# RupertLuo/Valley

Hardware: NVIDIA H100
Metric: generated tokens/s (8-frame video requests: ViT-L/14 encode + pool/project + LLaMA prefill + 256 greedy tokens per sequence) (higher is better)
Workload: dtype bf16

## Files before the change

valley_b200/csrc/api.cu:

```cuda
#include <cuda_runtime.h>
#include <cuda.h>

#include <algorithm>
#include <atomic>
#include <cmath>
#include <cstdarg>
#include <cstdio>
#include <cstdlib>
#include <cstring>
#include <map>
#include <memory>
#include <mutex>
#include <string>
#include <type_traits>
#include <utility>
#include <vector>

#include "../../include/valley_b200.h"
#include "attention_tc.cuh"
#include "common.cuh"
#include "gemm_tc.cuh"
#include "simt_kernels.cuh"
#include "decode_kernels.cuh"
#include "decode_mega.cuh"
// ... 166 lines not shown
  Owned<float> part_o;
  Owned<float2> part_ml;
  Owned<unsigned int> counters;
  Owned<float> part_val;
  Owned<int> part_idx;
  Owned<float> logits;
  Owned<long long> cur_tokens;
  Owned<long long> gen_tokens;
  int nsplit = 1;
  Owned<PhaseDesc> d_phases;
  StepParams mega = {};
  size_t mega_smem = 0;
  Owned<long long> dbg;
  Owned<SampleState> d_sample;
  bool sample_dirty = false;
  bool filtered = false;
  bool recording = false;
  Owned<uint32_t> key_bits;
  bool masked = false;
  int mask_words() const { return Smax / 32; }
  Owned<BeamState> d_beam;
  Owned<long long> beam_tok;
  Owned<int> beam_bidx;
  Owned<float> beam_div;
  Owned<int> beam_from;
  Owned<uint8_t> stop_buf, stop_stage;
  cudaEvent_t stop_event = nullptr;
  bool stop_ready = false;
  Owned<int> hist;
  bool procs_ready = false;
  StepGraphs graphs[kStepKinds];
  size_t layer_stride() const { return (size_t)2 * B * ctx->cfg.num_attention_heads * Smax * 128; }
  bf16* k_layer(int l) const { return cache + (size_t)l * layer_stride(); }
  bf16* v_layer(int l) const { return k_layer(l) + layer_stride() / 2; }

  ~vly_kv() {
    if (len_event) cudaEventDestroy(len_event);
    if (stop_event) cudaEventDestroy(stop_event);
  }
};

static int sync_len(vly_kv* kv) {
  if (!kv->len_dirty) return VLY_OK;
  CK(cudaSetDevice(kv->ctx->cfg.device));
  CK(cudaEventSynchronize(kv->len_event));
  kv->host_len = *reinterpret_cast<volatile int*>(kv->h_len.p);
  kv->len_dirty = false;
  return VLY_OK;
}

static inline int cdiv(long long a, long long b) { return int((a + b - 1) / b); }

static std::mutex g_attr_mu;
static std::map<std::pair<int, const void*>, size_t> g_attr_set;
template <typename Kern>
static int ensure_smem_attr(int device, Kern kern, size_t bytes, bool max_carveout) {
  std::lock_guard<std::mutex> lk(g_attr_mu);
  size_t& have = g_attr_set[std::make_pair(device, (const void*)kern)];
  if (bytes > have || (have == 0 && max_carveout)) {
    if (bytes > 0) CK(cudaFuncSetAttribute(kern, cudaFuncAttributeMaxDynamicSharedMemorySize, (int)bytes));
    if (max_carveout) CK(cudaFuncSetAttribute(kern, cudaFuncAttributePreferredSharedMemoryCarveout, 100));
    have = bytes > 0 ? bytes : 1;
  }
  return VLY_OK;
}

static int make_tmap_2d(vly_ctx* c, CUtensorMap* m, const void* ptr, uint64_t inner, uint64_t rows, uint64_t row_stride_bytes,
                        uint32_t box_inner, uint32_t box_rows, bool swizzle128 = true) {
  cuuint64_t dims[2] = {inner, rows};
  cuuint64_t strides[1] = {row_stride_bytes};
  cuuint32_t box[2] = {box_inner, box_rows};
  cuuint32_t es[2] = {1, 1};
  CUresult r = c->encode(m, CU_TENSOR_MAP_DATA_TYPE_BFLOAT16, 2, const_cast<void*>(ptr), dims, strides, box, es,
                         CU_TENSOR_MAP_INTERLEAVE_NONE, swizzle128 ? CU_TENSOR_MAP_SWIZZLE_128B : CU_TENSOR_MAP_SWIZZLE_NONE,
                         CU_TENSOR_MAP_L2_PROMOTION_L2_256B, CU_TENSOR_MAP_FLOAT_OOB_FILL_NONE);
  if (r != CUDA_SUCCESS)
    return fail(VLY_ERR_CUDA, "cuTensorMapEncodeTiled(2d) failed: %d (ptr=%p inner=%llu rows=%llu stride=%llu box=%u,%u)", (int)r, ptr,
                (unsigned long long)inner, (unsigned long long)rows, (unsigned long long)row_stride_bytes, box_inner, box_rows);
  return VLY_OK;
}
static int make_tmap_3d(vly_ctx* c, CUtensorMap* m, const void* ptr, uint64_t d0, uint64_t d1, uint64_t d2, uint64_t s1, uint64_t s2,
                        uint32_t b0, uint32_t b1) {
  cuuint64_t dims[3] = {d0, d1, d2};
  cuuint64_t strides[2] = {s1, s2};
  cuuint32_t box[3] = {b0, b1, 1};
  cuuint32_t es[3] = {1, 1, 1};
  CUresult r = c->encode(m, CU_TENSOR_MAP_DATA_TYPE_BFLOAT16, 3, const_cast<void*>(ptr), dims, strides, box, es,
                         CU_TENSOR_MAP_INTERLEAVE_NONE, CU_TENSOR_MAP_SWIZZLE_128B, CU_TENSOR_MAP_L2_PROMOTION_L2_256B,
                         CU_TENSOR_MAP_FLOAT_OOB_FILL_NONE);
  if (r != CUDA_SUCCESS) return fail(VLY_ERR_CUDA, "cuTensorMapEncodeTiled(3d) failed: %d", (int)r);
  return VLY_OK;
}

static bool pdl_enabled() {
  static const bool on = getenv("VLY_NO_PDL") == nullptr;
  return on;
}
struct LaunchCfg {
  dim3 grid, block;
  size_t smem = 0;
  cudaStream_t st = 0;
  bool pdl = false;
  bool carveout = false;
  bool cooperative = false;
};
template <typename... KArgs, typename... Args>
static int launch(vly_ctx* c, void (*kern)(KArgs...), const LaunchCfg& l, Args&&... args) {
  if (l.smem > 0 || l.carveout) TRY(ensure_smem_attr(c->cfg.device, kern, l.smem, l.carveout));
  cudaLaunchAttribute attr[2];
  unsigned n = 0;
  if (l.pdl && pdl_enabled()) {
    attr[n].id = cudaLaunchAttributeProgrammaticStreamSerialization;
    attr[n++].val.programmaticStreamSerializationAllowed = 1;
  }
  if (l.cooperative) {
    attr[n].id = cudaLaunchAttributeCooperative;
    attr[n++].val.cooperative = 1;
  }
  cudaLaunchConfig_t cfg = {};
  cfg.gridDim = l.grid;
  cfg.blockDim = l.block;
  cfg.dynamicSmemBytes = l.smem;
  cfg.stream = l.st;
  cfg.attrs = attr;
  cfg.numAttrs = n;
  const cudaError_t e = cudaLaunchKernelEx(&cfg, kern, std::forward<Args>(args)...);
  c->launches++;
  if (e != cudaSuccess) {
    cudaGetLastError();
    const char* name = "kernel";
    cudaFuncGetName(&name, (const void*)kern);
    return fail(VLY_ERR_CUDA, "launch of %s failed: %s", name, cudaGetErrorString(e));
  }
  return VLY_OK;
}

static inline int bmax_of(int B) { return B <= 1 ? 1 : (B <= 2 ? 2 : 4); }
template <typename F>
static int with_bmax(int B, F&& f) {
  if (bmax_of(B) == 1) return f(std::integral_constant<int, 1>());
  if (bmax_of(B) == 2) return f(std::integral_constant<int, 2>());
  return f(std::integral_constant<int, 4>());
}
template <typename T>
struct Type { using type = T; };
template <typename F>
static int with_dtype(int dtype, F&& f) {
  if (dtype == VLY_F32) return f(Type<float>());
  if (dtype == VLY_BF16) return f(Type<bf16>());
  if (dtype == VLY_F16) return f(Type<__half>());
  return fail(VLY_ERR_INVALID, "unknown dtype %d", dtype);
}

template <int BN, int EPI>
static int launch_gemm_t(vly_ctx* c, const bf16* A, long long lda, const bf16* W, long long ldw, GemmParams p, cudaStream_t st) {
  using Cfg = GemmCfg<BN>;
  CUtensorMap ta, tb;
  TRY(make_tmap_2d(c, &ta, A, p.K, p.M, lda * 2, 64, 128));
  TRY(make_tmap_2d(c, &tb, W, p.K, p.N, ldw * 2, 64, BN));
  p.num_m_tiles = cdiv(p.M, 128);
  p.num_n_tiles = cdiv(p.N, BN);
  const int tiles = p.num_m_tiles * p.num_n_tiles;
  return launch(c, gemm_tc_kernel<BN, EPI>, {dim3(tiles), dim3(Cfg::THREADS), Cfg::SMEM_BYTES, st, true}, ta, tb, p);
}
template <int EPI>
static int launch_gemm(vly_ctx* c, int bn, const bf16* A, long long lda, const bf16* W, long long ldw, const GemmParams& p,
                       cudaStream_t st) {
  if (bn == 256) return launch_gemm_t<256, EPI>(c, A, lda, W, ldw, p, st);
  return launch_gemm_t<128, EPI>(c, A, lda, W, ldw, p, st);
}
static inline int pick_bn(int N) { return (N % 256 == 0) ? 256 : 128; }
static inline int pick_bn_m(const vly_ctx* c, int N, int M) {
  if (N % 256 != 0) return 128;
  static const int env_bn = getenv("VLY_GEMM_BN") ? atoi(getenv("VLY_GEMM_BN")) : 0;
  if (env_bn == 128 || env_bn == 256) return env_bn;
  const long long t256 = (long long)cdiv(M, 128) * (N / 256), t128 = 2 * t256;
  if (t256 >= 3LL * c->num_sms) return 256;
  const double e256 = (double)t256 / ((double)cdiv(t256, c->num_sms) * c->num_sms);
  const double e128 = (double)t128 / ((double)cdiv(t128, c->num_sms) * c->num_sms);
  return (e128 > e256 * 1.05) ? 128 : 256;
}

__global__ void pack_rows_kernel(const bf16* __restrict__ src, int K, const float* __restrict__ gamma, const float* __restrict__ beta,
                                 const float* __restrict__ bias_in, bf16* __restrict__ dst, int Kdst, int mode, int off,
                                 float* __restrict__ colsum, float* __restrict__ bias_out) {
  __shared__ float r1[8], r2[8];
  const int r = blockIdx.x;
  int dr;
  if (mode == 0) dr = off + r;
  else if (mode == 1) {
    const int h = r >> 7, d = r & 127;
    dr = off + h * 128 + (d < 64 ? 2 * d : 2 * (d - 64) + 1);
  } else dr = 2 * r + off;
  float cs = 0.f, bb = 0.f;
  for (int k = threadIdx.x; k < Kdst; k += blockDim.x) {
    float wf = 0.f;
    if (k < K) {
      const float w = __bfloat162float(src[(size_t)r * K + k]);
      wf = gamma ? bf16_round(w * gamma[k]) : w;
      if (beta) bb += w * beta[k];
    }
    dst[(size_t)dr * Kdst + k] = __float2bfloat16_rn(wf);
    cs += wf;
  }
  cs = warp_sum(cs);
  bb = warp_sum(bb);
  if ((threadIdx.x & 31) == 0) {
    r1[threadIdx.x >> 5] = cs;
    r2[threadIdx.x >> 5] = bb;
  }
  __syncthreads();
  if (threadIdx.x == 0) {
    float a = 0.f, b = 0.f;
    for (int i = 0; i < (int)(blockDim.x >> 5); ++i) {
      a += r1[i];
      b += r2[i];
    }
    if (colsum) colsum[dr] = a;
    if (bias_out) bias_out[dr] = (bias_in ? bias_in[r] : 0.f) + b;
  }
}

__global__ void rope_table_kernel(float2* rope, int max_pos, float theta, int head_dim) {
  const int i = blockIdx.x * blockDim.x + threadIdx.x;
  const int half = head_dim / 2;
  if (i >= max_pos * half) return;
  const int pos = i / half, j = i % half;
  const float inv = 1.0f / powf(theta, float(2 * j) / float(head_dim));
  const float fr = float(pos) * inv;
  rope[i] = make_float2(bf16_round(cosf(fr)), bf16_round(sinf(fr)));
}

__global__ void set_int_kernel(int* p, int v) { *p = v; }

__global__ void __launch_bounds__(128) copy_rows_stats_kernel(const bf16* __restrict__ in, bf16* __restrict__ out,
                                                              float2* __restrict__ stats, int stats_nt, int H) {
  __shared__ float red[4];
  const int row = blockIdx.x;
  float s = 0.f, sq = 0.f;
  for (int c = threadIdx.x * 8; c < H; c += 128 * 8) {
    const uint4 w = *reinterpret_cast<const uint4*>(in + (size_t)row * H + c);
    *reinterpret_cast<uint4*>(out + (size_t)row * H + c) = w;
    const uint32_t ww[4] = {w.x, w.y, w.z, w.w};
#pragma unroll
    for (int i = 0; i < 4; ++i) {
      const float a = bf16_lo(ww[i]), b = bf16_hi(ww[i]);
      s += a + b;
      sq += a * a + b * b;
    }
  }
  s = block_sum_128(s, red);
  sq = block_sum_128(sq, red);
  if (threadIdx.x < stats_nt) stats[(size_t)row * stats_nt + threadIdx.x] = threadIdx.x == 0 ? make_float2(s, sq) : make_float2(0.f, 0.f);
}

__global__ void kv_export_kernel(const bf16* __restrict__ cache, bf16* __restrict__ out, int Smax, int len, int deinterleave) {
  const int bh = blockIdx.y, s = blockIdx.x, c = threadIdx.x;
  const int d = deinterleave ? ((c & 1) ? 64 + (c >> 1) : (c >> 1)) : c;
  out[((size_t)bh * len + s) * 128 + d] = cache[((size_t)bh * Smax + s) * 128 + c];
}

extern "C" int vly_create(const vly_config* cfg, vly_ctx** out) {
  if (!cfg || !out) return fail(VLY_ERR_INVALID, "vly_create: null argument");
  int ndev = 0;
  if (cudaGetDeviceCount(&ndev) != cudaSuccess || ndev == 0)
    return fail(VLY_ERR_CUDA, "vly_create: no CUDA device visible -- this library has no CPU fallback");
  CK(cudaSetDevice(cfg->device));
  cudaDeviceProp prop;
  CK(cudaGetDeviceProperties(&prop, cfg->device));
  if (prop.major != 9) return fail(VLY_ERR_CUDA, "vly_create: device is sm_%d%d; this library is built for sm_90a only", prop.major, prop.minor);
  if (cfg->hidden_size % 128 || cfg->hidden_size / cfg->num_attention_heads != 128)
    return fail(VLY_ERR_INVALID, "vly_create: head_dim must be 128 (hidden %d, heads %d)", cfg->hidden_size, cfg->num_attention_heads);
  if (cfg->intermediate_size % 64) return fail(VLY_ERR_INVALID, "vly_create: intermediate_size must be a multiple of 64");
  if (cfg->vit_hidden != 1024 || cfg->vit_hidden / cfg->vit_heads != 64 || cfg->vit_mlp % 256)
    return fail(VLY_ERR_INVALID, "vly_create: vision tower must be ViT-L width (1024, head_dim 64); the reference hard-codes 1024 (valley_model.py:192)");
  auto c = std::make_unique<vly_ctx>();
  c->cfg = *cfg;
  c->num_sms = prop.multiProcessorCount;
  cudaDriverEntryPointQueryResult qres;
  void* fn = nullptr;
  if (cudaGetDriverEntryPoint("cuTensorMapEncodeTiled", &fn, cudaEnableDefault, &qres) != cudaSuccess || fn == nullptr)
    return fail(VLY_ERR_CUDA, "vly_create: cuTensorMapEncodeTiled entry point not found");
  c->encode = (PFN_encodeTiled)fn;
  if (cudaStreamCreateWithFlags(&c->cap_stream, cudaStreamNonBlocking) != cudaSuccess)
    return fail(VLY_ERR_CUDA, "vly_create: cudaStreamCreate failed");
  *out = c.release();
  return VLY_OK;
}

extern "C" void vly_destroy(vly_ctx* c) {
  if (!c) return;
  cudaSetDevice(c->cfg.device);
  delete c;
}

extern "C" int vly_num_sms(vly_ctx* c, int* out) {
  if (!c || !out) return fail(VLY_ERR_INVALID, "null");
  *out = c->num_sms;
  return VLY_OK;
}
extern "C" int vly_kernel_launch_count(vly_ctx* c, int64_t* out) {
  if (!c || !out) return fail(VLY_ERR_INVALID, "null");
  std::lock_guard<std::mutex> lk(c->mu);
  *out = c->launches;
  return VLY_OK;
}
extern "C" int vly_held_bytes(int64_t* device_bytes, int64_t* pinned_bytes) {
  if (!device_bytes || !pinned_bytes) return fail(VLY_ERR_INVALID, "null");
  *device_bytes = g_held_bytes[0];
  *pinned_bytes = g_held_bytes[1];
  return VLY_OK;
}

static bool ends_with(const std::string& s, const char* suf) {
  const size_t n = strlen(suf);
  return s.size() >= n && s.compare(s.size() - n, n, suf) == 0;
}

extern "C" int vly_load_weight(vly_ctx* c, const char* name, const void* dev_ptr, int dtype, const int64_t* shape, int ndim) {
  if (!c || !name || !dev_ptr || !shape || ndim < 1 || ndim > 4) return fail(VLY_ERR_INVALID, "vly_load_weight: bad argument");
  std::lock_guard<std::mutex> lk(c->mu);
  if (c->finalized) return fail(VLY_ERR_STATE, "vly_load_weight(%s): weights already finalised", name);
  if (dtype != VLY_F32 && dtype != VLY_BF16 && dtype != VLY_F16)
    return fail(VLY_ERR_INVALID, "vly_load_weight(%s): unknown dtype %d", name, dtype);
  CK(cudaSetDevice(c->cfg.device));
  Staged s;
  s.numel = 1;
  for (int i = 0; i < ndim; ++i) {
    s.shape.push_back(shape[i]);
    s.numel *= shape[i];
  }
  const std::string nm(name);
  s.is_f32 = (ndim == 1) || ends_with(nm, "position_embedding.weight");
// ... 1596 lines not shown
```

valley_b200/csrc/gemm_tc.cuh:

```cuda
#pragma once
#include "common.cuh"
#include "wgmma.cuh"

namespace vly {

enum EpiMode : int {
  EPI_BIAS = 0,
  EPI_LN_BIAS = 1,
  EPI_LN_BIAS_GELU = 2,
  EPI_BIAS_RES_STATS = 3,
  EPI_RMS_QKV_ROPE = 4,
  EPI_RMS_SWIGLU = 5,
  EPI_RMS_F32 = 6,
};

struct GemmParams {
  int M, N, K;
  int num_m_tiles, num_n_tiles;
  void* out;
  long long ldo;
  const float* bias;
  const float* colsum;
  const float2* stats_in;
  int stats_in_nt;
  float inv_dim;
  float eps;
  float2* stats_out;
  const __nv_bfloat16* residual;
  long long ldr;
  const float2* rope;
  int S, past, H, nH, Smax;
  __nv_bfloat16* kcache;
  __nv_bfloat16* vcache;
  __nv_bfloat16* peer_out[8];
  int n_peers;
  int peer_tokens, peer_frame_stride;
  long long peer_frame_off;
};

VLY_DEVINL float tanh_approx(float x) {
  float y;
  asm("tanh.approx.f32 %0, %1;" : "=f"(y) : "f"(x));
  return y;
}
VLY_DEVINL float quick_gelu_f(float v) {
  const float h = 0.5f * v;
  return fmaf(h, tanh_approx(0.851f * v), h);
}
VLY_DEVINL float silu_f(float v) {
  const float h = 0.5f * v;
  return fmaf(h, tanh_approx(h), h);
}

template <int BN>
struct GemmCfg {
  static_assert(BN == 128 || BN == 256, "tile width");
  static constexpr int BM = 128, BK = 64;
  static constexpr int STAGES = (BN == 256) ? 4 : 6;
  static constexpr int A_BYTES = BM * BK * 2;
  static constexpr int B_BYTES = BN * BK * 2;
  static constexpr int STAGE_BYTES = A_BYTES + B_BYTES;
  static constexpr int RING_BYTES = STAGES * STAGE_BYTES;
  static constexpr int ACC_LD = BN + 4;
  static_assert(BM * ACC_LD * 4 <= RING_BYTES, "accumulator staging must fit in the drained ring");
  static constexpr int VEC_BYTES = 2  * BN * 4;
  static constexpr int SMEM_BYTES = RING_BYTES + 1024  + 256  + VEC_BYTES;
  static constexpr int THREADS = 384;
};

template <int BN, int EPI>
__global__ void __launch_bounds__(384, 1)
gemm_tc_kernel(const __grid_constant__ CUtensorMap tma_a, const __grid_constant__ CUtensorMap tma_b, const GemmParams p) {
  using Cfg = GemmCfg<BN>;
  constexpr int BM = Cfg::BM, BK = Cfg::BK, STAGES = Cfg::STAGES;
  extern __shared__ uint8_t smem_raw[];
  const uint32_t base_u32 = (smem_u32(smem_raw) + 1023u) & ~1023u;
  uint8_t* smem = smem_raw + (base_u32 - smem_u32(smem_raw));
  uint8_t* sA = smem;
  uint8_t* sB = smem + STAGES * Cfg::A_BYTES;
  uint64_t* bars = reinterpret_cast<uint64_t*>(smem + Cfg::RING_BYTES);
  uint64_t* full_bar = bars;
  uint64_t* empty_bar = bars + STAGES;
  float* sbias = reinterpret_cast<float*>(smem + Cfg::RING_BYTES + 256);
  float* scol = sbias + BN;

  const int wg = threadIdx.x >> 7;
  const int num_kb = (p.K + BK - 1) / BK;
  const int m_blk = (int)blockIdx.x / p.num_n_tiles, n_blk = (int)blockIdx.x % p.num_n_tiles;

  if (threadIdx.x == 0) {
    tma_prefetch_desc(&tma_a);
    tma_prefetch_desc(&tma_b);
    for (int i = 0; i < STAGES; ++i) {
      mbar_init(&full_bar[i], 1);
      mbar_init(&empty_bar[i], 256);
    }
    fence_barrier_init();
  }
  __syncthreads();
  pdl_launch_dependents();

  if (wg == 0) {
    if (threadIdx.x == 0) {
      pdl_wait();
      int stage = 0;
      uint32_t phase = 0;
      for (int kb = 0; kb < num_kb; ++kb) {
        mbar_wait(&empty_bar[stage], phase ^ 1);
        mbar_expect_tx(&full_bar[stage], Cfg::STAGE_BYTES);
        tma_load_2d(sA + stage * Cfg::A_BYTES, &tma_a, &full_bar[stage], kb * BK, m_blk * BM);
        tma_load_2d(sB + stage * Cfg::B_BYTES, &tma_b, &full_bar[stage], kb * BK, n_blk * BN);
        if (++stage == STAGES) { stage = 0; phase ^= 1; }
      }
    }
    return;
  }

  const int ct = threadIdx.x - 128;
  const int t = threadIdx.x & 127;
  const int row0 = (wg - 1) * 64;
  constexpr int NB = BN / 128;
  float acc[NB][64];
#pragma unroll
  for (int nb = 0; nb < NB; ++nb)
#pragma unroll
    for (int i = 0; i < 64; ++i) acc[nb][i] = 0.f;
  {
    int stage = 0, prev = -1;
    uint32_t phase = 0;
    for (int kb = 0; kb < num_kb; ++kb) {
      mbar_wait(&full_bar[stage], phase);
      const uint64_t da = make_smem_desc_sw128(base_u32 + stage * Cfg::A_BYTES + row0 * 128, 16, 1024);
      const uint64_t db = make_smem_desc_sw128(base_u32 + STAGES * Cfg::A_BYTES + stage * Cfg::B_BYTES, 16, 1024);
      wgmma_fence();
#pragma unroll
      for (int k = 0; k < BK / 16; ++k)
#pragma unroll
        for (int nb = 0; nb < NB; ++nb)
          wgmma_ss_n128(acc[nb], da + 2 * k, db + 2 * k + nb * 1024, (kb | k) != 0);
      wgmma_commit();
      wgmma_wait<1>();
      if (prev >= 0) mbar_arrive(&empty_bar[prev]);
      prev = stage;
      if (++stage == STAGES) { stage = 0; phase ^= 1; }
    }
    wgmma_wait<0>();
#pragma unroll
    for (int nb = 0; nb < NB; ++nb) wgmma_fence_regs(acc[nb]);
  }

  pdl_wait();
  constexpr bool kHasVec = (EPI == EPI_BIAS || EPI == EPI_BIAS_RES_STATS || EPI == EPI_LN_BIAS || EPI == EPI_LN_BIAS_GELU);
  if constexpr (kHasVec) {
    for (int i = ct; i < BN; i += 256) {
      const int n = n_blk * BN + i;
      sbias[i] = (p.bias != nullptr && n < p.N) ? __ldg(p.bias + n) : 0.f;
      if constexpr (EPI == EPI_LN_BIAS || EPI == EPI_LN_BIAS_GELU) scol[i] = (n < p.N) ? __ldg(p.colsum + n) : 0.f;
    }
  }
  asm volatile("bar.sync 1, 256;" ::: "memory");
  float* stg = reinterpret_cast<float*>(smem);
  {
    const int w = t >> 5, l = t & 31;
    const int r = row0 + w * 16 + (l >> 2), c0 = (l & 3) * 2;
#pragma unroll
    for (int nb = 0; nb < NB; ++nb)
#pragma unroll
      for (int j = 0; j < 16; ++j) {
        const int col = nb * 128 + j * 8 + c0;
        *reinterpret_cast<float2*>(stg + (size_t)r * Cfg::ACC_LD + col) = make_float2(acc[nb][4 * j], acc[nb][4 * j + 1]);
        *reinterpret_cast<float2*>(stg + (size_t)(r + 8) * Cfg::ACC_LD + col) = make_float2(acc[nb][4 * j + 2], acc[nb][4 * j + 3]);
      }
  }
  asm volatile("bar.sync %0, 128;" ::"r"(1 + wg) : "memory");

  const int r_in_tile = row0 + (t >> 1);
  const int hf = t & 1;
  const int row = m_blk * BM + r_in_tile;
  const bool row_ok = row < p.M;

  float mean = 0.f, rstd = 1.f;
  if constexpr (EPI == EPI_LN_BIAS || EPI == EPI_LN_BIAS_GELU || EPI == EPI_RMS_QKV_ROPE || EPI == EPI_RMS_SWIGLU ||
                EPI == EPI_RMS_F32) {
    if (row_ok) {
      float s = 0.f, ss = 0.f;
      const float2* st = p.stats_in + (size_t)row * p.stats_in_nt;
      for (int i = 0; i < p.stats_in_nt; ++i) {
        const float2 v = st[i];
        s += v.x;
        ss += v.y;
      }
      if constexpr (EPI == EPI_LN_BIAS || EPI == EPI_LN_BIAS_GELU) {
        mean = s * p.inv_dim;
        const float var = fmaxf(ss * p.inv_dim - mean * mean, 0.f);
        rstd = rsqrtf(var + p.eps);
      } else {
        rstd = rsqrtf(ss * p.inv_dim + p.eps);
      }
    }
  }
  int b_idx = 0, pos = 0;
  if constexpr (EPI == EPI_RMS_QKV_ROPE) {
    if (row_ok) {
      b_idx = row / p.S;
      pos = p.past + (row % p.S);
    }
  }
  float st_sum = 0.f, st_sq = 0.f;
  long long peer_row = 0;
  if constexpr (EPI == EPI_BIAS_RES_STATS) {
    if (p.n_peers > 0) {
      const int f = row / p.peer_tokens;
      peer_row = (p.peer_frame_off + (long long)f * p.peer_frame_stride) * p.peer_tokens + (row - f * p.peer_tokens);
    }
  }
  const float* srow = stg + (size_t)r_in_tile * Cfg::ACC_LD;
  auto process_chunk = [&](const int c) {
    const int n0 = n_blk * BN + c * 32;
    if (row_ok && n0 < p.N) {
    float v[32];
#pragma unroll
    for (int i = 0; i < 32; i += 4) {
      const float4 a4 = *reinterpret_cast<const float4*>(srow + c * 32 + i);
      v[i] = a4.x; v[i + 1] = a4.y; v[i + 2] = a4.z; v[i + 3] = a4.w;
    }

    if constexpr (EPI == EPI_BIAS || EPI == EPI_BIAS_RES_STATS) {
      const float4* b4 = reinterpret_cast<const float4*>(sbias + c * 32);
#pragma unroll
      for (int j = 0; j < 8; ++j) {
        const float4 bb = b4[j];
        v[4 * j] += bb.x; v[4 * j + 1] += bb.y; v[4 * j + 2] += bb.z; v[4 * j + 3] += bb.w;
      }
    }
    if constexpr (EPI == EPI_LN_BIAS || EPI == EPI_LN_BIAS_GELU) {
      const float4* b4 = reinterpret_cast<const float4*>(sbias + c * 32);
      const float4* c4 = reinterpret_cast<const float4*>(scol + c * 32);
      const float nm = -mean * rstd;
#pragma unroll
      for (int j = 0; j < 8; ++j) {
        const float4 bb = b4[j], cc = c4[j];
        const float bq[4] = {bb.x, bb.y, bb.z, bb.w}, cq[4] = {cc.x, cc.y, cc.z, cc.w};
#pragma unroll
        for (int t4 = 0; t4 < 4; ++t4) {
          float t = fmaf(rstd, v[4 * j + t4], fmaf(nm, cq[t4], bq[t4]));
          if constexpr (EPI == EPI_LN_BIAS_GELU) t = quick_gelu_f(t);
          v[4 * j + t4] = t;
        }
      }
    }
    if constexpr (EPI == EPI_RMS_QKV_ROPE || EPI == EPI_RMS_SWIGLU || EPI == EPI_RMS_F32) {
#pragma unroll
      for (int i = 0; i < 32; ++i) v[i] *= rstd;
    }

    if constexpr (EPI == EPI_BIAS_RES_STATS) {
      uint4 o[4];
      const uint4* rp = reinterpret_cast<const uint4*>(p.residual + (size_t)row * p.ldr + n0);
#pragma unroll
      for (int j = 0; j < 4; ++j) {
        const uint4 rr = __ldg(rp + j);
        const uint32_t rw[4] = {rr.x, rr.y, rr.z, rr.w};
        uint32_t ow[4];
#pragma unroll
        for (int t = 0; t < 4; ++t) {
          const float a = v[j * 8 + t * 2] + bf16_lo(rw[t]);
          const float b = v[j * 8 + t * 2 + 1] + bf16_hi(rw[t]);
          ow[t] = pack_bf16x2(a, b);
          const float ar = bf16_lo(ow[t]), br = bf16_hi(ow[t]);
          st_sum += ar + br;
          st_sq += ar * ar + br * br;
        }
        o[j] = make_uint4(ow[0], ow[1], ow[2], ow[3]);
      }
      uint4* op = reinterpret_cast<uint4*>(reinterpret_cast<__nv_bfloat16*>(p.out) + (size_t)row * p.ldo + n0);
#pragma unroll
      for (int j = 0; j < 4; ++j) op[j] = o[j];
      if (p.n_peers > 0) {
        for (int q = 0; q < p.n_peers; ++q) {
          uint4* pp = reinterpret_cast<uint4*>(p.peer_out[q] + (size_t)peer_row * p.ldo + n0);
#pragma unroll
          for (int j = 0; j < 4; ++j) pp[j] = o[j];
        }
      }
    } else if constexpr (EPI == EPI_RMS_SWIGLU) {
      uint32_t ow[8];
#pragma unroll
      for (int j = 0; j < 8; ++j) {
        const float a = silu_f(v[4 * j]) * v[4 * j + 1];
        const float b = silu_f(v[4 * j + 2]) * v[4 * j + 3];
        ow[j] = pack_bf16x2(a, b);
      }
      uint4* op = reinterpret_cast<uint4*>(reinterpret_cast<__nv_bfloat16*>(p.out) + (size_t)row * p.ldo + (n0 >> 1));
      op[0] = make_uint4(ow[0], ow[1], ow[2], ow[3]);
      op[1] = make_uint4(ow[4], ow[5], ow[6], ow[7]);
    } else if constexpr (EPI == EPI_RMS_F32) {
      float* op = reinterpret_cast<float*>(p.out) + (size_t)row * p.ldo + n0;
      if (n0 + 32 <= p.N && (p.ldo & 3) == 0) {
#pragma unroll
        for (int j = 0; j < 8; ++j)
          reinterpret_cast<float4*>(op)[j] = make_float4(v[4 * j], v[4 * j + 1], v[4 * j + 2], v[4 * j + 3]);
      } else {
#pragma unroll
        for (int i = 0; i < 32; ++i)
          if (n0 + i < p.N) op[i] = v[i];
      }
    } else if constexpr (EPI == EPI_RMS_QKV_ROPE) {
      const int which = n0 / p.H;
      const int nh = n0 - which * p.H;
      const int head = nh >> 7, cidx = nh & 127;
      if (which < 2) {
        const float2* cs = p.rope + (size_t)pos * 64 + (cidx >> 1);
#pragma unroll
        for (int j = 0; j < 16; ++j) {
          const float2 c_s = __ldg(cs + j);
          const float x0 = v[2 * j], x1 = v[2 * j + 1];
          v[2 * j] = x0 * c_s.x - x1 * c_s.y;
          v[2 * j + 1] = x1 * c_s.x + x0 * c_s.y;
        }
      }
      __nv_bfloat16* dst;
      if (which == 0) {
        dst = reinterpret_cast<__nv_bfloat16*>(p.out) + (size_t)row * p.ldo + nh;
      } else {
        __nv_bfloat16* cache = (which == 1) ? p.kcache : p.vcache;
        dst = cache + (((size_t)b_idx * p.nH + head) * p.Smax + pos) * 128 + cidx;
      }
      uint4* op = reinterpret_cast<uint4*>(dst);
#pragma unroll
      for (int j = 0; j < 4; ++j)
        op[j] = make_uint4(pack_bf16x2(v[8 * j], v[8 * j + 1]), pack_bf16x2(v[8 * j + 2], v[8 * j + 3]),
                           pack_bf16x2(v[8 * j + 4], v[8 * j + 5]), pack_bf16x2(v[8 * j + 6], v[8 * j + 7]));
    } else {
      __nv_bfloat16* dst = reinterpret_cast<__nv_bfloat16*>(p.out) + (size_t)row * p.ldo + n0;
      if (n0 + 32 <= p.N && (p.ldo & 7) == 0) {
        uint4* op = reinterpret_cast<uint4*>(dst);
#pragma unroll
        for (int j = 0; j < 4; ++j)
          op[j] = make_uint4(pack_bf16x2(v[8 * j], v[8 * j + 1]), pack_bf16x2(v[8 * j + 2], v[8 * j + 3]),
                             pack_bf16x2(v[8 * j + 4], v[8 * j + 5]), pack_bf16x2(v[8 * j + 6], v[8 * j + 7]));
      } else {
#pragma unroll
        for (int i = 0; i < 32; ++i)
          if (n0 + i < p.N) dst[i] = __float2bfloat16_rn(v[i]);
      }
    }
    }
  };
  constexpr int CPT = BN / 64;
#pragma unroll
  for (int cc = 0; cc < CPT; ++cc) process_chunk(hf * CPT + cc);
  if constexpr (EPI == EPI_BIAS_RES_STATS) {
    st_sum += __shfl_xor_sync(0xffffffffu, st_sum, 1);
    st_sq += __shfl_xor_sync(0xffffffffu, st_sq, 1);
    if (hf == 0 && row_ok && p.stats_out != nullptr) p.stats_out[(size_t)row * p.num_n_tiles + n_blk] = make_float2(st_sum, st_sq);
  }
}

}
```

Before: 388.2.

## Make tensor-core GEMM persistent with ping-pong consumer warpgroups and banded tile order

```diff
diff --git a/valley_b200/csrc/api.cu b/valley_b200/csrc/api.cu
--- a/valley_b200/csrc/api.cu
+++ b/valley_b200/csrc/api.cu
@@ -342,16 +342,26 @@
   return fail(VLY_ERR_INVALID, "unknown dtype %d", dtype);
 }
 
+static bool gemm_one_tile_per_cta() {
+  const char* e = getenv("VLY_GEMM_ONE_TILE");
+  return e != nullptr && atoi(e) != 0;
+}
+static inline int gemm_tiles(int M, int N, int bn) { return cdiv(M, GemmCfg<128>::BM) * cdiv(N, bn); }
+static inline int gemm_grid(const vly_ctx* c, int tiles) {
+  return gemm_one_tile_per_cta() ? cdiv(tiles, 2) : std::min(tiles, c->num_sms);
+}
 template <int BN, int EPI>
 static int launch_gemm_t(vly_ctx* c, const bf16* A, long long lda, const bf16* W, long long ldw, GemmParams p, cudaStream_t st) {
   using Cfg = GemmCfg<BN>;
   CUtensorMap ta, tb;
-  TRY(make_tmap_2d(c, &ta, A, p.K, p.M, lda * 2, 64, 128));
+  TRY(make_tmap_2d(c, &ta, A, p.K, p.M, lda * 2, 64, Cfg::BM));
   TRY(make_tmap_2d(c, &tb, W, p.K, p.N, ldw * 2, 64, BN));
-  p.num_m_tiles = cdiv(p.M, 128);
+  p.num_m_tiles = cdiv(p.M, Cfg::BM);
   p.num_n_tiles = cdiv(p.N, BN);
-  const int tiles = p.num_m_tiles * p.num_n_tiles;
-  return launch(c, gemm_tc_kernel<BN, EPI>, {dim3(tiles), dim3(Cfg::THREADS), Cfg::SMEM_BYTES, st, true}, ta, tb, p);
+  const long long a_row_block = (long long)Cfg::BM * p.K * 2, a_band = 24LL << 20;
+  p.band_m = (p.M > p.N && p.num_m_tiles * a_row_block > a_band) ? (int)std::max(1LL, a_band / a_row_block) : p.num_m_tiles;
+  const int grid = gemm_grid(c, p.num_m_tiles * p.num_n_tiles);
+  return launch(c, gemm_tc_kernel<BN, EPI>, {dim3(grid), dim3(Cfg::THREADS), Cfg::SMEM_BYTES, st, true}, ta, tb, p);
 }
 template <int EPI>
 static int launch_gemm(vly_ctx* c, int bn, const bf16* A, long long lda, const bf16* W, long long ldw, const GemmParams& p,
@@ -364,11 +374,9 @@
   if (N % 256 != 0) return 128;
   static const int env_bn = getenv("VLY_GEMM_BN") ? atoi(getenv("VLY_GEMM_BN")) : 0;
   if (env_bn == 128 || env_bn == 256) return env_bn;
-  const long long t256 = (long long)cdiv(M, 128) * (N / 256), t128 = 2 * t256;
-  if (t256 >= 3LL * c->num_sms) return 256;
-  const double e256 = (double)t256 / ((double)cdiv(t256, c->num_sms) * c->num_sms);
-  const double e128 = (double)t128 / ((double)cdiv(t128, c->num_sms) * c->num_sms);
-  return (e128 > e256 * 1.05) ? 128 : 256;
+  if (gemm_tiles(M, N, 256) < c->num_sms) return 256;
+  const long long w256 = 2LL * cdiv(gemm_tiles(M, N, 256), c->num_sms), w128 = cdiv(gemm_tiles(M, N, 128), c->num_sms);
+  return (w128 * 8 < w256 * 7) ? 128 : 256;
 }
 
 __global__ void pack_rows_kernel(const bf16* __restrict__ src, int K, const float* __restrict__ gamma, const float* __restrict__ beta,
diff --git a/valley_b200/csrc/gemm_tc.cuh b/valley_b200/csrc/gemm_tc.cuh
--- a/valley_b200/csrc/gemm_tc.cuh
+++ b/valley_b200/csrc/gemm_tc.cuh
@@ -17,6 +17,7 @@
 struct GemmParams {
   int M, N, K;
   int num_m_tiles, num_n_tiles;
+  int band_m;
   void* out;
   long long ldo;
   const float* bias;
@@ -55,18 +56,30 @@
 template <int BN>
 struct GemmCfg {
   static_assert(BN == 128 || BN == 256, "tile width");
-  static constexpr int BM = 128, BK = 64;
-  static constexpr int STAGES = (BN == 256) ? 4 : 6;
+  static constexpr int BM = 64, BK = 64;
   static constexpr int A_BYTES = BM * BK * 2;
   static constexpr int B_BYTES = BN * BK * 2;
   static constexpr int STAGE_BYTES = A_BYTES + B_BYTES;
+  static constexpr int ACC_LD = 128 + 4;
+  static constexpr int STG_BYTES = BM * ACC_LD * 4;
+  static constexpr int VEC_BYTES = 2  * BN * 4;
+  static constexpr int FIXED_BYTES = 1024  + 256  + STG_BYTES + VEC_BYTES;
+  static constexpr int MAX_SMEM = 227 * 1024;
+  static constexpr int STAGES = (MAX_SMEM - FIXED_BYTES) / STAGE_BYTES;
   static constexpr int RING_BYTES = STAGES * STAGE_BYTES;
-  static constexpr int ACC_LD = BN + 4;
-  static_assert(BM * ACC_LD * 4 <= RING_BYTES, "accumulator staging must fit in the drained ring");
-  static constexpr int VEC_BYTES = 2  * BN * 4;
-  static constexpr int SMEM_BYTES = RING_BYTES + 1024  + 256  + VEC_BYTES;
+  static_assert(2 * STAGES * 8 <= 256, "barriers");
+  static constexpr int SMEM_BYTES = RING_BYTES + FIXED_BYTES;
   static constexpr int THREADS = 384;
 };
+
+VLY_DEVINL void tile_mn(const GemmParams& p, int tile, int& m_blk, int& n_blk) {
+  const int per_band = p.band_m * p.num_n_tiles, band = tile / per_band, in_band = tile - band * per_band;
+  const int rows = min(p.band_m, p.num_m_tiles - band * p.band_m);
+  m_blk = band * p.band_m + in_band % rows;
+  n_blk = in_band / rows;
+}
+VLY_DEVINL void named_bar_sync(int id, int n) { asm volatile("bar.sync %0, %1;" ::"r"(id), "r"(n) : "memory"); }
+VLY_DEVINL void named_bar_arrive(int id, int n) { asm volatile("bar.arrive %0, %1;" ::"r"(id), "r"(n) : "memory"); }
 
 template <int BN, int EPI>
 __global__ void __launch_bounds__(384, 1)
@@ -81,19 +94,20 @@
   uint64_t* bars = reinterpret_cast<uint64_t*>(smem + Cfg::RING_BYTES);
   uint64_t* full_bar = bars;
   uint64_t* empty_bar = bars + STAGES;
-  float* sbias = reinterpret_cast<float*>(smem + Cfg::RING_BYTES + 256);
+  float* stg = reinterpret_cast<float*>(smem + Cfg::RING_BYTES + 256);
+  float* sbias = stg + BM * Cfg::ACC_LD;
   float* scol = sbias + BN;
 
   const int wg = threadIdx.x >> 7;
   const int num_kb = (p.K + BK - 1) / BK;
-  const int m_blk = (int)blockIdx.x / p.num_n_tiles, n_blk = (int)blockIdx.x % p.num_n_tiles;
+  const int num_tiles = p.num_m_tiles * p.num_n_tiles;
 
   if (threadIdx.x == 0) {
     tma_prefetch_desc(&tma_a);
     tma_prefetch_desc(&tma_b);
     for (int i = 0; i < STAGES; ++i) {
       mbar_init(&full_bar[i], 1);
-      mbar_init(&empty_bar[i], 256);
+      mbar_init(&empty_bar[i], 128);
     }
     fence_barrier_init();
   }
@@ -105,255 +119,271 @@
       pdl_wait();
       int stage = 0;
       uint32_t phase = 0;
-      for (int kb = 0; kb < num_kb; ++kb) {
-        mbar_wait(&empty_bar[stage], phase ^ 1);
-        mbar_expect_tx(&full_bar[stage], Cfg::STAGE_BYTES);
-        tma_load_2d(sA + stage * Cfg::A_BYTES, &tma_a, &full_bar[stage], kb * BK, m_blk * BM);
-        tma_load_2d(sB + stage * Cfg::B_BYTES, &tma_b, &full_bar[stage], kb * BK, n_blk * BN);
-        if (++stage == STAGES) { stage = 0; phase ^= 1; }
+      for (int tile = blockIdx.x; tile < num_tiles; tile += gridDim.x) {
+        int m_blk, n_blk;
+        tile_mn(p, tile, m_blk, n_blk);
+        for (int kb = 0; kb < num_kb; ++kb) {
+          mbar_wait(&empty_bar[stage], phase ^ 1);
+          mbar_expect_tx(&full_bar[stage], Cfg::STAGE_BYTES);
+          tma_load_2d(sA + stage * Cfg::A_BYTES, &tma_a, &full_bar[stage], kb * BK, m_blk * BM);
+          tma_load_2d(sB + stage * Cfg::B_BYTES, &tma_b, &full_bar[stage], kb * BK, n_blk * BN);
+          if (++stage == STAGES) { stage = 0; phase ^= 1; }
+        }
       }
     }
     return;
   }
 
-  const int ct = threadIdx.x - 128;
+  const int w = wg - 1;
   const int t = threadIdx.x & 127;
-  const int row0 = (wg - 1) * 64;
   constexpr int NB = BN / 128;
-  float acc[NB][64];
-#pragma unroll
-  for (int nb = 0; nb < NB; ++nb)
-#pragma unroll
-    for (int i = 0; i < 64; ++i) acc[nb][i] = 0.f;
-  {
-    int stage = 0, prev = -1;
-    uint32_t phase = 0;
-    for (int kb = 0; kb < num_kb; ++kb) {
-      mbar_wait(&full_bar[stage], phase);
-      const uint64_t da = make_smem_desc_sw128(base_u32 + stage * Cfg::A_BYTES + row0 * 128, 16, 1024);
-      const uint64_t db = make_smem_desc_sw128(base_u32 + STAGES * Cfg::A_BYTES + stage * Cfg::B_BYTES, 16, 1024);
-      wgmma_fence();
-#pragma unroll
-      for (int k = 0; k < BK / 16; ++k)
-#pragma unroll
-        for (int nb = 0; nb < NB; ++nb)
-          wgmma_ss_n128(acc[nb], da + 2 * k, db + 2 * k + nb * 1024, (kb | k) != 0);
-      wgmma_commit();
-      wgmma_wait<1>();
-      if (prev >= 0) mbar_arrive(&empty_bar[prev]);
-      prev = stage;
-      if (++stage == STAGES) { stage = 0; phase ^= 1; }
-    }
-    wgmma_wait<0>();
-#pragma unroll
-    for (int nb = 0; nb < NB; ++nb) wgmma_fence_regs(acc[nb]);
-  }
-
-  pdl_wait();
-  constexpr bool kHasVec = (EPI == EPI_BIAS || EPI == EPI_BIAS_RES_STATS || EPI == EPI_LN_BIAS || EPI == EPI_LN_BIAS_GELU);
-  if constexpr (kHasVec) {
-    for (int i = ct; i < BN; i += 256) {
-      const int n = n_blk * BN + i;
-      sbias[i] = (p.bias != nullptr && n < p.N) ? __ldg(p.bias + n) : 0.f;
-      if constexpr (EPI == EPI_LN_BIAS || EPI == EPI_LN_BIAS_GELU) scol[i] = (n < p.N) ? __ldg(p.colsum + n) : 0.f;
-    }
-  }
-  asm volatile("bar.sync 1, 256;" ::: "memory");
-  float* stg = reinterpret_cast<float*>(smem);
-  {
-    const int w = t >> 5, l = t & 31;
-    const int r = row0 + w * 16 + (l >> 2), c0 = (l & 3) * 2;
+  constexpr int CPT = BN / 64;
+  for (int i = w;; i += 2) {
+    const int tile = (int)blockIdx.x + i * (int)gridDim.x;
+    if (tile >= num_tiles) break;
+    int m_blk, n_blk;
+    tile_mn(p, tile, m_blk, n_blk);
+    float acc[NB][64];
 #pragma unroll
     for (int nb = 0; nb < NB; ++nb)
 #pragma unroll
-      for (int j = 0; j < 16; ++j) {
-        const int col = nb * 128 + j * 8 + c0;
-        *reinterpret_cast<float2*>(stg + (size_t)r * Cfg::ACC_LD + col) = make_float2(acc[nb][4 * j], acc[nb][4 * j + 1]);
-        *reinterpret_cast<float2*>(stg + (size_t)(r + 8) * Cfg::ACC_LD + col) = make_float2(acc[nb][4 * j + 2], acc[nb][4 * j + 3]);
-      }
-  }
-  asm volatile("bar.sync %0, 128;" ::"r"(1 + wg) : "memory");
-
-  const int r_in_tile = row0 + (t >> 1);
-  const int hf = t & 1;
-  const int row = m_blk * BM + r_in_tile;
-  const bool row_ok = row < p.M;
-
-  float mean = 0.f, rstd = 1.f;
-  if constexpr (EPI == EPI_LN_BIAS || EPI == EPI_LN_BIAS_GELU || EPI == EPI_RMS_QKV_ROPE || EPI == EPI_RMS_SWIGLU ||
-                EPI == EPI_RMS_F32) {
-    if (row_ok) {
-      float s = 0.f, ss = 0.f;
-      const float2* st = p.stats_in + (size_t)row * p.stats_in_nt;
-      for (int i = 0; i < p.stats_in_nt; ++i) {
-        const float2 v = st[i];
-        s += v.x;
-        ss += v.y;
+      for (int j = 0; j < 64; ++j) acc[nb][j] = 0.f;
+    if (i > 0) named_bar_sync(5 + (w ^ 1), 256);
+    {
+      const int pos0 = i * num_kb;
+      int stage = pos0 % STAGES, prev = -1;
+      uint32_t phase = (uint32_t)(pos0 / STAGES) & 1u;
+      for (int kb = 0; kb < num_kb; ++kb) {
+        mbar_wait(&full_bar[stage], phase);
+        const uint64_t da = make_smem_desc_sw128(base_u32 + stage * Cfg::A_BYTES, 16, 1024);
+        const uint64_t db = make_smem_desc_sw128(base_u32 + STAGES * Cfg::A_BYTES + stage * Cfg::B_BYTES, 16, 1024);
+        wgmma_fence();
+#pragma unroll
+        for (int k = 0; k < BK / 16; ++k)
+#pragma unroll
+          for (int nb = 0; nb < NB; ++nb)
+            wgmma_ss_n128(acc[nb], da + 2 * k, db + 2 * k + nb * 1024, (kb | k) != 0);
+        wgmma_commit();
+        wgmma_wait<1>();
+        if (prev >= 0) mbar_arrive(&empty_bar[prev]);
+        prev = stage;
+        if (++stage == STAGES) { stage = 0; phase ^= 1; }
+      }
+      if (tile + (int)gridDim.x < num_tiles) named_bar_arrive(5 + w, 256);
+      wgmma_wait<0>();
+      mbar_arrive(&empty_bar[prev]);
+#pragma unroll
+      for (int nb = 0; nb < NB; ++nb) wgmma_fence_regs(acc[nb]);
+    }
+
+    pdl_wait();
+    if (i > 0) named_bar_sync(3 + (w ^ 1), 256);
+    constexpr bool kHasVec = (EPI == EPI_BIAS || EPI == EPI_BIAS_RES_STATS || EPI == EPI_LN_BIAS || EPI == EPI_LN_BIAS_GELU);
+    if constexpr (kHasVec) {
+      for (int j = t; j < BN; j += 128) {
+        const int n = n_blk * BN + j;
+        sbias[j] = (p.bias != nullptr && n < p.N) ? __ldg(p.bias + n) : 0.f;
+        if constexpr (EPI == EPI_LN_BIAS || EPI == EPI_LN_BIAS_GELU) scol[j] = (n < p.N) ? __ldg(p.colsum + n) : 0.f;
+      }
+    }
+
+    const int r_in_tile = t >> 1;
+    const int hf = t & 1;
+    const int row = m_blk * BM + r_in_tile;
+    const bool row_ok = row < p.M;
+
+    float mean = 0.f, rstd = 1.f;
+    if constexpr (EPI == EPI_LN_BIAS || EPI == EPI_LN_BIAS_GELU || EPI == EPI_RMS_QKV_ROPE || EPI == EPI_RMS_SWIGLU ||
+                  EPI == EPI_RMS_F32) {
+      if (row_ok) {
+        float s = 0.f, ss = 0.f;
+        const float2* st = p.stats_in + (size_t)row * p.stats_in_nt;
+        for (int i = 0; i < p.stats_in_nt; ++i) {
+          const float2 v = st[i];
+          s += v.x;
+          ss += v.y;
+        }
+        if constexpr (EPI == EPI_LN_BIAS || EPI == EPI_LN_BIAS_GELU) {
+          mean = s * p.inv_dim;
+          const float var = fmaxf(ss * p.inv_dim - mean * mean, 0.f);
+          rstd = rsqrtf(var + p.eps);
+        } else {
+          rstd = rsqrtf(ss * p.inv_dim + p.eps);
+        }
+      }
+    }
+    int b_idx = 0, pos = 0;
+    if constexpr (EPI == EPI_RMS_QKV_ROPE) {
+      if (row_ok) {
+        b_idx = row / p.S;
+        pos = p.past + (row % p.S);
+      }
+    }
+    float st_sum = 0.f, st_sq = 0.f;
+    long long peer_row = 0;
+    if constexpr (EPI == EPI_BIAS_RES_STATS) {
+      if (p.n_peers > 0) {
+        const int f = row / p.peer_tokens;
+        peer_row = (p.peer_frame_off + (long long)f * p.peer_frame_stride) * p.peer_tokens + (row - f * p.peer_tokens);
+      }
+    }
+    const float* srow = stg + (size_t)r_in_tile * Cfg::ACC_LD;
+    auto process_chunk = [&](const int c) {
+      const int n0 = n_blk * BN + c * 32;
+      if (row_ok && n0 < p.N) {
+      float v[32];
+#pragma unroll
+      for (int i = 0; i < 32; i += 4) {
+        const float4 a4 = *reinterpret_cast<const float4*>(srow + (c & 3) * 32 + i);
+        v[i] = a4.x; v[i + 1] = a4.y; v[i + 2] = a4.z; v[i + 3] = a4.w;
+      }
+
+      if constexpr (EPI == EPI_BIAS || EPI == EPI_BIAS_RES_STATS) {
+        const float4* b4 = reinterpret_cast<const float4*>(sbias + c * 32);
+#pragma unroll
+        for (int j = 0; j < 8; ++j) {
+          const float4 bb = b4[j];
+          v[4 * j] += bb.x; v[4 * j + 1] += bb.y; v[4 * j + 2] += bb.z; v[4 * j + 3] += bb.w;
+        }
       }
       if constexpr (EPI == EPI_LN_BIAS || EPI == EPI_LN_BIAS_GELU) {
-        mean = s * p.inv_dim;
-        const float var = fmaxf(ss * p.inv_dim - mean * mean, 0.f);
-        rstd = rsqrtf(var + p.eps);
-      } else {
-        rstd = rsqrtf(ss * p.inv_dim + p.eps);
-      }
-    }
-  }
-  int b_idx = 0, pos = 0;
-  if constexpr (EPI == EPI_RMS_QKV_ROPE) {
-    if (row_ok) {
-      b_idx = row / p.S;
-      pos = p.past + (row % p.S);
-    }
-  }
-  float st_sum = 0.f, st_sq = 0.f;
-  long long peer_row = 0;
-  if constexpr (EPI == EPI_BIAS_RES_STATS) {
-    if (p.n_peers > 0) {
-      const int f = row / p.peer_tokens;
-      peer_row = (p.peer_frame_off + (long long)f * p.peer_frame_stride) * p.peer_tokens + (row - f * p.peer_tokens);
-    }
-  }
-  const float* srow = stg + (size_t)r_in_tile * Cfg::ACC_LD;
-  auto process_chunk = [&](const int c) {
-    const int n0 = n_blk * BN + c * 32;
-    if (row_ok && n0 < p.N) {
-    float v[32];
-#pragma unroll
-    for (int i = 0; i < 32; i += 4) {
-      const float4 a4 = *reinterpret_cast<const float4*>(srow + c * 32 + i);
-      v[i] = a4.x; v[i + 1] = a4.y; v[i + 2] = a4.z; v[i + 3] = a4.w;
-    }
-
-    if constexpr (EPI == EPI_BIAS || EPI == EPI_BIAS_RES_STATS) {
-      const float4* b4 = reinterpret_cast<const float4*>(sbias + c * 32);
-#pragma unroll
-      for (int j = 0; j < 8; ++j) {
-        const float4 bb = b4[j];
-        v[4 * j] += bb.x; v[4 * j + 1] += bb.y; v[4 * j + 2] += bb.z; v[4 * j + 3] += bb.w;
-      }
-    }
-    if constexpr (EPI == EPI_LN_BIAS || EPI == EPI_LN_BIAS_GELU) {
-      const float4* b4 = reinterpret_cast<const float4*>(sbias + c * 32);
-      const float4* c4 = reinterpret_cast<const float4*>(scol + c * 32);
-      const float nm = -mean * rstd;
-#pragma unroll
-      for (int j = 0; j < 8; ++j) {
-        const float4 bb = b4[j], cc = c4[j];
-        const float bq[4] = {bb.x, bb.y, bb.z, bb.w}, cq[4] = {cc.x, cc.y, cc.z, cc.w};
-#pragma unroll
-        for (int t4 = 0; t4 < 4; ++t4) {
-          float t = fmaf(rstd, v[4 * j + t4], fmaf(nm, cq[t4], bq[t4]));
-          if constexpr (EPI == EPI_LN_BIAS_GELU) t = quick_gelu_f(t);
-          v[4 * j + t4] = t;
-        }
-      }
-    }
-    if constexpr (EPI == EPI_RMS_QKV_ROPE || EPI == EPI_RMS_SWIGLU || EPI == EPI_RMS_F32) {
-#pragma unroll
-      for (int i = 0; i < 32; ++i) v[i] *= rstd;
-    }
-
-    if constexpr (EPI == EPI_BIAS_RES_STATS) {
-      uint4 o[4];
-      const uint4* rp = reinterpret_cast<const uint4*>(p.residual + (size_t)row * p.ldr + n0);
-#pragma unroll
-      for (int j = 0; j < 4; ++j) {
-        const uint4 rr = __ldg(rp + j);
-        const uint32_t rw[4] = {rr.x, rr.y, rr.z, rr.w};
-        uint32_t ow[4];
-#pragma unroll
-        for (int t = 0; t < 4; ++t) {
-          const float a = v[j * 8 + t * 2] + bf16_lo(rw[t]);
-          const float b = v[j * 8 + t * 2 + 1] + bf16_hi(rw[t]);
-          ow[t] = pack_bf16x2(a, b);
-          const float ar = bf16_lo(ow[t]), br = bf16_hi(ow[t]);
-          st_sum += ar + br;
-          st_sq += ar * ar + br * br;
-        }
-        o[j] = make_uint4(ow[0], ow[1], ow[2], ow[3]);
-      }
-      uint4* op = reinterpret_cast<uint4*>(reinterpret_cast<__nv_bfloat16*>(p.out) + (size_t)row * p.ldo + n0);
-#pragma unroll
-      for (int j = 0; j < 4; ++j) op[j] = o[j];
-      if (p.n_peers > 0) {
-        for (int q = 0; q < p.n_peers; ++q) {
-          uint4* pp = reinterpret_cast<uint4*>(p.peer_out[q] + (size_t)peer_row * p.ldo + n0);
-#pragma unroll
-          for (int j = 0; j < 4; ++j) pp[j] = o[j];
-        }
-      }
-    } else if constexpr (EPI == EPI_RMS_SWIGLU) {
-      uint32_t ow[8];
-#pragma unroll
-      for (int j = 0; j < 8; ++j) {
-        const float a = silu_f(v[4 * j]) * v[4 * j + 1];
-        const float b = silu_f(v[4 * j + 2]) * v[4 * j + 3];
-        ow[j] = pack_bf16x2(a, b);
-      }
-      uint4* op = reinterpret_cast<uint4*>(reinterpret_cast<__nv_bfloat16*>(p.out) + (size_t)row * p.ldo + (n0 >> 1));
-      op[0] = make_uint4(ow[0], ow[1], ow[2], ow[3]);
-      op[1] = make_uint4(ow[4], ow[5], ow[6], ow[7]);
-    } else if constexpr (EPI == EPI_RMS_F32) {
-      float* op = reinterpret_cast<float*>(p.out) + (size_t)row * p.ldo + n0;
-      if (n0 + 32 <= p.N && (p.ldo & 3) == 0) {
-#pragma unroll
-        for (int j = 0; j < 8; ++j)
-          reinterpret_cast<float4*>(op)[j] = make_float4(v[4 * j], v[4 * j + 1], v[4 * j + 2], v[4 * j + 3]);
-      } else {
-#pragma unroll
-        for (int i = 0; i < 32; ++i)
-          if (n0 + i < p.N) op[i] = v[i];
-      }
-    } else if constexpr (EPI == EPI_RMS_QKV_ROPE) {
-      const int which = n0 / p.H;
-      const int nh = n0 - which * p.H;
-      const int head = nh >> 7, cidx = nh & 127;
-      if (which < 2) {
-        const float2* cs = p.rope + (size_t)pos * 64 + (cidx >> 1);
-#pragma unroll
-        for (int j = 0; j < 16; ++j) {
-          const float2 c_s = __ldg(cs + j);
-          const float x0 = v[2 * j], x1 = v[2 * j + 1];
-          v[2 * j] = x0 * c_s.x - x1 * c_s.y;
-          v[2 * j + 1] = x1 * c_s.x + x0 * c_s.y;
-        }
-      }
-      __nv_bfloat16* dst;
-      if (which == 0) {
-        dst = reinterpret_cast<__nv_bfloat16*>(p.out) + (size_t)row * p.ldo + nh;
-      } else {
-        __nv_bfloat16* cache = (which == 1) ? p.kcache : p.vcache;
-        dst = cache + (((size_t)b_idx * p.nH + head) * p.Smax + pos) * 128 + cidx;
-      }
-      uint4* op = reinterpret_cast<uint4*>(dst);
-#pragma unroll
-      for (int j = 0; j < 4; ++j)
-        op[j] = make_uint4(pack_bf16x2(v[8 * j], v[8 * j + 1]), pack_bf16x2(v[8 * j + 2], v[8 * j + 3]),
-                           pack_bf16x2(v[8 * j + 4], v[8 * j + 5]), pack_bf16x2(v[8 * j + 6], v[8 * j + 7]));
-    } else {
-      __nv_bfloat16* dst = reinterpret_cast<__nv_bfloat16*>(p.out) + (size_t)row * p.ldo + n0;
-      if (n0 + 32 <= p.N && (p.ldo & 7) == 0) {
+        const float4* b4 = reinterpret_cast<const float4*>(sbias + c * 32);
+        const float4* c4 = reinterpret_cast<const float4*>(scol + c * 32);
+        const float nm = -mean * rstd;
+#pragma unroll
+        for (int j = 0; j < 8; ++j) {
+          const float4 bb = b4[j], cc = c4[j];
+          const float bq[4] = {bb.x, bb.y, bb.z, bb.w}, cq[4] = {cc.x, cc.y, cc.z, cc.w};
+#pragma unroll
+          for (int t4 = 0; t4 < 4; ++t4) {
+            float t = fmaf(rstd, v[4 * j + t4], fmaf(nm, cq[t4], bq[t4]));
+            if constexpr (EPI == EPI_LN_BIAS_GELU) t = quick_gelu_f(t);
+            v[4 * j + t4] = t;
+          }
+        }
+      }
+      if constexpr (EPI == EPI_RMS_QKV_ROPE || EPI == EPI_RMS_SWIGLU || EPI == EPI_RMS_F32) {
+#pragma unroll
+        for (int i = 0; i < 32; ++i) v[i] *= rstd;
+      }
+
+      if constexpr (EPI == EPI_BIAS_RES_STATS) {
+        uint4 o[4];
+        const uint4* rp = reinterpret_cast<const uint4*>(p.residual + (size_t)row * p.ldr + n0);
+#pragma unroll
+        for (int j = 0; j < 4; ++j) {
+          const uint4 rr = __ldg(rp + j);
+          const uint32_t rw[4] = {rr.x, rr.y, rr.z, rr.w};
+          uint32_t ow[4];
+#pragma unroll
+          for (int t = 0; t < 4; ++t) {
+            const float a = v[j * 8 + t * 2] + bf16_lo(rw[t]);
+            const float b = v[j * 8 + t * 2 + 1] + bf16_hi(rw[t]);
+            ow[t] = pack_bf16x2(a, b);
+            const float ar = bf16_lo(ow[t]), br = bf16_hi(ow[t]);
+            st_sum += ar + br;
+            st_sq += ar * ar + br * br;
+          }
+          o[j] = make_uint4(ow[0], ow[1], ow[2], ow[3]);
+        }
+        uint4* op = reinterpret_cast<uint4*>(reinterpret_cast<__nv_bfloat16*>(p.out) + (size_t)row * p.ldo + n0);
+#pragma unroll
+        for (int j = 0; j < 4; ++j) op[j] = o[j];
+        if (p.n_peers > 0) {
+          for (int q = 0; q < p.n_peers; ++q) {
+            uint4* pp = reinterpret_cast<uint4*>(p.peer_out[q] + (size_t)peer_row * p.ldo + n0);
+#pragma unroll
+            for (int j = 0; j < 4; ++j) pp[j] = o[j];
+          }
+        }
+      } else if constexpr (EPI == EPI_RMS_SWIGLU) {
+        uint32_t ow[8];
+#pragma unroll
+        for (int j = 0; j < 8; ++j) {
+          const float a = silu_f(v[4 * j]) * v[4 * j + 1];
+          const float b = silu_f(v[4 * j + 2]) * v[4 * j + 3];
+          ow[j] = pack_bf16x2(a, b);
+        }
+        uint4* op = reinterpret_cast<uint4*>(reinterpret_cast<__nv_bfloat16*>(p.out) + (size_t)row * p.ldo + (n0 >> 1));
+        op[0] = make_uint4(ow[0], ow[1], ow[2], ow[3]);
+        op[1] = make_uint4(ow[4], ow[5], ow[6], ow[7]);
+      } else if constexpr (EPI == EPI_RMS_F32) {
+        float* op = reinterpret_cast<float*>(p.out) + (size_t)row * p.ldo + n0;
+        if (n0 + 32 <= p.N && (p.ldo & 3) == 0) {
+#pragma unroll
+          for (int j = 0; j < 8; ++j)
+            reinterpret_cast<float4*>(op)[j] = make_float4(v[4 * j], v[4 * j + 1], v[4 * j + 2], v[4 * j + 3]);
+        } else {
+#pragma unroll
+          for (int i = 0; i < 32; ++i)
+            if (n0 + i < p.N) op[i] = v[i];
+        }
+      } else if constexpr (EPI == EPI_RMS_QKV_ROPE) {
+        const int which = n0 / p.H;
+        const int nh = n0 - which * p.H;
+        const int head = nh >> 7, cidx = nh & 127;
+        if (which < 2) {
+          const float2* cs = p.rope + (size_t)pos * 64 + (cidx >> 1);
+#pragma unroll
+          for (int j = 0; j < 16; ++j) {
+            const float2 c_s = __ldg(cs + j);
+            const float x0 = v[2 * j], x1 = v[2 * j + 1];
+            v[2 * j] = x0 * c_s.x - x1 * c_s.y;
+            v[2 * j + 1] = x1 * c_s.x + x0 * c_s.y;
+          }
+        }
+        __nv_bfloat16* dst;
+        if (which == 0) {
+          dst = reinterpret_cast<__nv_bfloat16*>(p.out) + (size_t)row * p.ldo + nh;
+        } else {
+          __nv_bfloat16* cache = (which == 1) ? p.kcache : p.vcache;
+          dst = cache + (((size_t)b_idx * p.nH + head) * p.Smax + pos) * 128 + cidx;
+        }
         uint4* op = reinterpret_cast<uint4*>(dst);
 #pragma unroll
         for (int j = 0; j < 4; ++j)
           op[j] = make_uint4(pack_bf16x2(v[8 * j], v[8 * j + 1]), pack_bf16x2(v[8 * j + 2], v[8 * j + 3]),
                              pack_bf16x2(v[8 * j + 4], v[8 * j + 5]), pack_bf16x2(v[8 * j + 6], v[8 * j + 7]));
       } else {
-#pragma unroll
-        for (int i = 0; i < 32; ++i)
-          if (n0 + i < p.N) dst[i] = __float2bfloat16_rn(v[i]);
-      }
-    }
-    }
-  };
-  constexpr int CPT = BN / 64;
-#pragma unroll
-  for (int cc = 0; cc < CPT; ++cc) process_chunk(hf * CPT + cc);
-  if constexpr (EPI == EPI_BIAS_RES_STATS) {
-    st_sum += __shfl_xor_sync(0xffffffffu, st_sum, 1);
-    st_sq += __shfl_xor_sync(0xffffffffu, st_sq, 1);
-    if (hf == 0 && row_ok && p.stats_out != nullptr) p.stats_out[(size_t)row * p.num_n_tiles + n_blk] = make_float2(st_sum, st_sq);
+        __nv_bfloat16* dst = reinterpret_cast<__nv_bfloat16*>(p.out) + (size_t)row * p.ldo + n0;
+        if (n0 + 32 <= p.N && (p.ldo & 7) == 0) {
+          uint4* op = reinterpret_cast<uint4*>(dst);
+#pragma unroll
+          for (int j = 0; j < 4; ++j)
+            op[j] = make_uint4(pack_bf16x2(v[8 * j], v[8 * j + 1]), pack_bf16x2(v[8 * j + 2], v[8 * j + 3]),
+                               pack_bf16x2(v[8 * j + 4], v[8 * j + 5]), pack_bf16x2(v[8 * j + 6], v[8 * j + 7]));
+        } else {
+#pragma unroll
+          for (int i = 0; i < 32; ++i)
+            if (n0 + i < p.N) dst[i] = __float2bfloat16_rn(v[i]);
+        }
+      }
+      }
+    };
+#pragma unroll
+    for (int nb = 0; nb < NB; ++nb) {
+      if (nb > 0) named_bar_sync(1 + w, 128);
+      {
+        const int wp = t >> 5, l = t & 31;
+        const int r = wp * 16 + (l >> 2), c0 = (l & 3) * 2;
+#pragma unroll
+        for (int j = 0; j < 16; ++j) {
+          const int col = j * 8 + c0;
+          *reinterpret_cast<float2*>(stg + (size_t)r * Cfg::ACC_LD + col) = make_float2(acc[nb][4 * j], acc[nb][4 * j + 1]);
+          *reinterpret_cast<float2*>(stg + (size_t)(r + 8) * Cfg::ACC_LD + col) = make_float2(acc[nb][4 * j + 2], acc[nb][4 * j + 3]);
+        }
+      }
+      named_bar_sync(1 + w, 128);
+#pragma unroll
+      for (int cc = 0; cc < CPT; ++cc)
+        if (((hf * CPT + cc) >> 2) == nb) process_chunk(hf * CPT + cc);
+    }
+    if constexpr (EPI == EPI_BIAS_RES_STATS) {
+      st_sum += __shfl_xor_sync(0xffffffffu, st_sum, 1);
+      st_sq += __shfl_xor_sync(0xffffffffu, st_sq, 1);
+      if (hf == 0 && row_ok && p.stats_out != nullptr) p.stats_out[(size_t)row * p.num_n_tiles + n_blk] = make_float2(st_sum, st_sq);
+    }
+    if (tile + (int)gridDim.x < num_tiles) named_bar_arrive(3 + w, 256);
   }
 }
 
```

Result: no change. 390.2 (median of 6 runs) (+0.5%).
